# AIM-Harvard/pyradiomics

Measured on AMD Instinct MI355X. Metric: Mvoxels/s for GLCM+GLRLM build, 512^3 vol @32 bins, higher is better.
Workload: dtype u8 levels / u32 counts / f64 out; 1 GPU; GLCM+GLRLM matrix build, 512^3 int32+uint8 volume resident in HBM, 32 grey levels, full mask, 13 angles, uniform levels; one volume per GPU (batch sharding, no collective); size=512, levels=32, dist=uniform, deferred_mode=pipeline

## Files before the change

pyradiomics_amd/csrc/kernels_sweep.h:

```cpp
#pragma once
#include "prad_runtime.h"

namespace prad {

typedef unsigned int u32;
typedef unsigned long long u64;

__global__ void __launch_bounds__(256) pack_levels_kernel(const int *__restrict__ image,
                                                          const uint8_t *__restrict__ mask, long long n, int NX,
                                                          int pitch, int padw, int Ng,
                                                          uint8_t *__restrict__ levels, int *__restrict__ flags,
                                                          int vec_ok, int shift, uint8_t *__restrict__ rowzero = nullptr) {
  const long long tid = (long long)blockIdx.x * blockDim.x + threadIdx.x;
  const long long nthreads = (long long)gridDim.x * blockDim.x;
  const bool linear = (padw == 0 && pitch == NX);
  int bad = 0;
  long long done = 0;
  if (vec_ok) {
    const long long n16 = n >> 4;
    const int upr = NX >> 4;
    const int4 *im4 = reinterpret_cast<const int4 *>(image);
    const uint4 *mk4 = reinterpret_cast<const uint4 *>(mask);
    for (long long t = tid; t < n16; t += nthreads) {
      const uint4 m = mk4[t];
// ... 305 lines not shown
}
template <int LPL, int U, typename W>
__device__ __forceinline__ void steps_plain_group(W (&w)[LPL], const unsigned (&v)[U]) {
#pragma unroll
  for (int k = 0; k < U; k++) step_lines_plain<LPL>(w, v[k]);
}
template <int LPL, int U, bool LONG>
__device__ __forceinline__ void steps_plain_group(Walker<true, true, LONG, true> (&w)[LPL], const unsigned (&v)[U]) {
  unsigned pw = pack_prev<LPL>(w);
#pragma unroll
  for (int k = 0; k < U; k++) {
    step_lines_plain<LPL, LONG>(w, v[k], pw);
    pw = v[k];
  }
  unpack_prev<LPL>(w, pw);
}

template <int LPL, int U, bool CHECK, typename W>
__device__ __forceinline__ bool steps_break_group(W (&w)[LPL], const unsigned (&v)[U], const int (&sb)[U],
                                                  const bool (&uw)[U], int lane4) {
  bool m = false;
#pragma unroll
  for (int k = 0; k < U; k++) {
#pragma unroll
    for (int j = 0; j < LPL; j++) {
      const bool brk = uw[k] || (sb[k] == lane4 + j);
      m |= w[j].template step_brk<CHECK>((int)((v[k] >> (8 * j)) & 0xffu), brk);
    }
  }
  return m;
}
template <bool DO_GLCM, bool DO_GLRLM, bool FUSED>
__device__ __forceinline__ void flush_block_hist(const u32 *lds, const HistLayout &h, int Nr, int slot,
                                                 u32 *__restrict__ glcm_acc, u32 *__restrict__ glrlm_acc) {
  __syncthreads();
  const int Ng = h.Ng;
  if (FUSED) {
    const int Q = Ng + 1, P = (h.RS + 1) * Q;
    u32 *gd = glcm_acc + (size_t)slot * Ng * Ng;
    for (int i = threadIdx.x; i < Ng * Ng; i += blockDim.x) {
      const int p = i / Ng, c = i - p * Ng;
      if (p == c) continue;
      u32 v = 0;
      for (int l = 0; l <= h.RS; l++) v += lds[(p + 1) * P + l * Q + c + 1];
      if (v) atomicAdd(gd + i, v);
    }
    u32 *rd = glrlm_acc + (size_t)slot * Ng * Nr;
    for (int i = threadIdx.x; i < Ng * h.RS; i += blockDim.x) {
      const int p = i / h.RS, l = i - p * h.RS;
      u32 v = 0;
      for (int c = 0; c <= Ng; c++) v += lds[(p + 1) * P + l * Q + c];
      if (v) atomicAdd(rd + (size_t)p * Nr + l, v);
    }
    for (int i = threadIdx.x; i < Ng * h.RL; i += blockDim.x) {
      const int p = i / h.RL, l = h.RS + (i - p * h.RL);
      const u32 v = lds[h.g0 + i];
      if (v && l < Nr) atomicAdd(rd + (size_t)p * Nr + l, v);
    }
    return;
  }
  if (DO_GLCM) {
    u32 *dst = glcm_acc + (size_t)slot * Ng * Ng;
    for (int i = threadIdx.x; i < Ng * Ng; i += blockDim.x) {
      const u32 v = lds[i];
      if (v) atomicAdd(dst + i, v);
    }
  }
  if (DO_GLRLM) {
    const u32 *hr = lds + h.glrlm0;
    u32 *dst = glrlm_acc + (size_t)slot * Ng * Nr;
    for (int i = threadIdx.x; i < h.RS * Ng; i += blockDim.x) {
      const u32 v = hr[i];
      if (v) atomicAdd(dst + (size_t)(i % Ng) * Nr + (i / Ng), v);
    }
  }
}

#ifndef PRAD_SWEEP_UNROLL
#define PRAD_SWEEP_UNROLL 8
#endif

struct __attribute__((packed)) u32_unaligned { u32 v; };
struct __attribute__((packed)) u16_unaligned { unsigned short v; };
template <int LPL>
__device__ __forceinline__ u32 load_lines(const uint8_t *p) {
#ifdef PRAD_DBG_NOLOAD
  const u32 x = (u32)(size_t)p * 2654435761u;
  return ((x >> 7) & 0x1f1f1f1fu) + 0x01010101u;
#else
  if (LPL == 4) return reinterpret_cast<const u32_unaligned *>(p)->v;
// ... 372 lines not shown
```

pyradiomics_amd/csrc/kernels_sweepfw.h:

```cpp
#pragma once
#include "kernels_sweep.h"

namespace prad {

enum FwPhase { FP_INIT, FP_GRAB, FP_CTRL, FP_ISSUE, FP_WAIT_ROWS, FP_WAIT_PACK, FP_GROUP, FP_PACK, FP_SLOW, FP_FLUSH, FP_DRAIN,
               FP_TOTAL, FP_REALTIME, FP_NGROUP, FP_NGROUP_PACK, FP_NSLOW, FP_COUNT };
#ifdef PRAD_FW_STAMPS
__device__ unsigned long long prad_fw_stamps[2 * 8192 * FP_COUNT];
struct FwClock {
  unsigned long long last, first, rt0;
  unsigned acc[FP_COUNT];
  __device__ __forceinline__ void start() {
#pragma unroll
    for (int i = 0; i < FP_COUNT; i++) acc[i] = 0;
    rt0 = __builtin_amdgcn_s_memrealtime();
    first = last = __builtin_readcyclecounter();
  }
  template <int PH>
  __device__ __forceinline__ void lap() {
    const unsigned long long now = __builtin_readcyclecounter();
    acc[PH] += (unsigned)(now - last);
    last = now;
  }
  template <int PH>
// ... 26 lines not shown
  long long sM, sU;
  int CL, pieces;
  int chunks;
  int dom_kind;
};
struct FwSet {
  int count;
  int NX;
  int pitch;
  int nrows;
  int xcd;
  int first_block[PRAD_MAX_SWEEP + 1];
  FwDesc d[PRAD_MAX_SWEEP];
};

struct PackJob {
  const int *image;
  const uint8_t *mask;
  uint8_t *levels;
  uint8_t *levels16;
  uint8_t *rowzero;
  int *flags;
  long long n16;
  int NX, Ng;
  int every;
};

#define PRAD_FW_U 8
#ifndef PRAD_FW_MAXG
#define PRAD_FW_MAXG 4
#endif
#define PRAD_FW_WORK_STRIDE 64
#define PRAD_FW_DOMAINS 8
__host__ __device__ inline size_t fw_lds_bytes(const HistLayout &h) { return 4 * ((size_t)h.words + (size_t)(h.Ng + 1)); }


struct FwTab {
  u32 *rl_long;
  int Nr, P4, Q, lenlim, gB, RL4, RS, RL, dummy0b, alive0, deadmax;
  unsigned Qinv;
  __device__ __forceinline__ void init(const HistLayout &h, int Nr_, u32 *rl_long_) {
    rl_long = rl_long_;
    Nr = Nr_;
    Q = 4 * (h.Ng + 1);
    P4 = (h.RS + 1) * (h.Ng + 1);
    lenlim = (h.RS + 1) * Q;
    RS = h.RS;
    RL = h.RL;
    RL4 = 4 * h.RL;
    gB = Q + 4 * h.g0 - RL4 - 4 * h.RS;
    Qinv = (unsigned)((0x100000000ull + (unsigned)Q - 1) / (unsigned)Q);
    dummy0b = Q + 4 * h.dummy0;
    alive0 = (h.RS + 2) * Q;
    deadmax = (h.RS + 1) * Q;
  }
};

__device__ __noinline__ void fw_long_event(const FwTab &T, int lv, int lb) {
  const int idx = (int)__umulhi((unsigned)lb, T.Qinv);
  if (idx < T.RS + T.RL) {
    lds_bump(T.gB + __mul24(lv, T.RL4) + (idx << 2));
    return;
  }
  const unsigned key = ((unsigned)lv << 20) | (unsigned)idx;
  bool pending = true;
  while (pending) {
// ... 757 lines not shown
      const uint4 *row = reinterpret_cast<const uint4 *>(tile + lane * PRAD_ROW_PITCH);
#pragma unroll
      for (int q = 0; q < 4; q++) {
        const uint4 d = row[q];
        const u32 wds[4] = {d.x, d.y, d.z, d.w};
        const unsigned m = (pw >> 24) ? (unsigned)(s - __mul24((int)(pw >> 24), T.P4)) : 0u;
        if (LONG && __ballot(m + 16 * T.Q > (unsigned)T.lenlim) != 0) {
#pragma unroll 1
          for (int k = 0; k < 4; k++) {
            const u32 c = wds[k], x = __builtin_amdgcn_alignbyte(c, pw, 3);
            const unsigned m4 = (pw >> 24) ? (unsigned)(s - __mul24((int)(pw >> 24), T.P4)) : 0u;
            if (__ballot(m4 + 4 * T.Q > (unsigned)T.lenlim) != 0) {
#pragma unroll
              for (int b = 0; b < 4; b++) fw_checked<LONG>(T, dummy, s, (int)((x >> (8 * b)) & 0xffu), (int)((c >> (8 * b)) & 0xffu), false);
            } else {
              fw_row_word<ZA>(T, one, s, c, x);
            }
            pw = c;
          }
        } else {
#pragma unroll
          for (int k = 0; k < 4; k++) {
            fw_row_word<ZA>(T, one, s, wds[k], __builtin_amdgcn_alignbyte(wds[k], pw, 3));
            pw = wds[k];
          }
        }
      }
      __builtin_amdgcn_wave_barrier();
    }
    fw_checked<LONG>(T, dummy, s, (int)(pw >> 24), 0, false);
  }
}

template <bool LONG>
__global__ void __launch_bounds__(1024) sweep_fw_rows_kernel(const uint8_t *__restrict__ L, long long nrows, int NX, int pitch,
                                                            int slot, int Ng, int Nr, int RS, u32 *__restrict__ glcm_acc,
                                                            u32 *__restrict__ glrlm_acc, int *__restrict__ flags) {
  extern __shared__ u32 lds[];
  if (flags[0]) return;
  const HistLayout h = hist_layout(true, true, true, Ng, RS);
  if ((unsigned)(size_t)((lds_u32 *)lds) != 0u) {
    if (threadIdx.x == 0) atomicExch(flags + 2, 1);
    return;
  }
  for (int i = threadIdx.x; i < h.words + Ng + 1; i += blockDim.x) lds[i] = 0;
  __syncthreads();
  FwTab T;
  T.init(h, Nr, glrlm_acc + (size_t)slot * Ng * Nr);
  if (flags[3] != 0) fw_rows_role<LONG, true>(h, T, lds, L, nrows, NX, pitch, (int)blockIdx.x, (int)gridDim.x);
  else fw_rows_role<LONG, false>(h, T, lds, L, nrows, NX, pitch, (int)blockIdx.x, (int)gridDim.x);
  flush_block_hist<true, true, true>(lds + Ng + 1, h, Nr, slot, glcm_acc, glrlm_acc);
}

template <bool LONG, int K, bool HASPAD, bool PACK>
__global__ void __launch_bounds__(1024) sweep_fw_kernel(FwSet set, PackJob pj, const uint8_t *__restrict__ L,
                                                        const uint8_t *__restrict__ rowzero, int Ng, int Nr, int RS,
                                                        u32 *__restrict__ glcm_acc, u32 *__restrict__ glrlm_acc,
                                                        int *__restrict__ work, int *__restrict__ flags) {
  extern __shared__ u32 lds[];
  int role = 0;
  while (role + 1 < set.count && (int)blockIdx.x >= set.first_block[role + 1]) role++;
  const int bx = (int)blockIdx.x - set.first_block[role], nblocks = set.first_block[role + 1] - set.first_block[role];
  const int wpb = (int)(blockDim.x >> 6);
  const long long pw = __builtin_amdgcn_readfirstlane((int)(blockIdx.x * wpb + (threadIdx.x >> 6)));
  PackWave pk(pj, pw, (long long)gridDim.x * wpb);
  FwClock clk;
  clk.start();
#ifdef PRAD_FW_SETPRIO
  __builtin_amdgcn_s_setprio(PRAD_FW_SETPRIO);
#endif
  if (flags[0] == 0) {
    const bool anyzero = flags[3] != 0;
    const HistLayout h = hist_layout(true, true, true, Ng, RS);
    if ((unsigned)(size_t)((lds_u32 *)lds) != 0u) {
      if (threadIdx.x == 0) atomicExch(flags + 2, 1);
    } else {
      for (int i = threadIdx.x; i < h.words + Ng + 1; i += blockDim.x) lds[i] = 0;
      __syncthreads();
      clk.lap<FP_INIT>();
      const FwDesc &D = set.d[role];
      FwTab T;
      T.init(h, Nr, glrlm_acc + (size_t)D.slot * Ng * Nr);
      int *wk = work + PRAD_FW_WORK_STRIDE * PRAD_FW_DOMAINS * role;
      if (D.dx == 0) {
        FwWave<LONG, K, 0, HASPAD, PACK> w(T, set.NX);
        w.run(D, set.NX, set.pitch, set.nrows, L, rowzero, anyzero, wk, bx, nblocks, pk, pj, set.xcd != 0, clk);
      } else if (D.dx > 0) {
        FwWave<LONG, K, 1, HASPAD, PACK> w(T, set.NX);
        w.run(D, set.NX, set.pitch, set.nrows, L, rowzero, anyzero, wk, bx, nblocks, pk, pj, set.xcd != 0, clk);
      } else {
        FwWave<LONG, K, -1, HASPAD, PACK> w(T, set.NX);
        w.run(D, set.NX, set.pitch, set.nrows, L, rowzero, anyzero, wk, bx, nblocks, pk, pj, set.xcd != 0, clk);
      }
      clk.lap<FP_CTRL>();
      flush_block_hist<true, true, true>(lds + Ng + 1, h, Nr, D.slot, glcm_acc, glrlm_acc);
      clk.lap<FP_FLUSH>();
    }
  }
  if (PACK) pk.drain(pj);
  clk.lap<FP_DRAIN>();
  clk.store(PACK ? 1 : 0);
}

}
```

pyradiomics_amd/csrc/prad_api.hip:

```cpp
#include "prad_runtime.h"
#include "kernels_generic.h"
#include "kernels_pairs.h"
#include "kernels_sweep.h"
#include "kernels_sweepfw.h"
#include "kernels_sweepfw2.h"
#include "kernels_neigh.h"
#include "kernels_glszm.h"
#include "kernels_voxel.h"
#include "kernels_voxslide.h"
#include "kernels_mcc.h"
#include "kernels_voxtex.h"
#include "kernels_binning.h"

#include <algorithm>
#include <atomic>
#include <chrono>
#include <cmath>
#include <condition_variable>
#include <cstdlib>
#include <deque>
#include <limits>
#include <mutex>
#include <thread>

// ... 571 lines not shown
int launch_fw2_khsp(Call &k, const SweepPlan &p, const PackJob &pj, const uint8_t *levels16, int Ng, int Nr, u32 *glcm_acc, u32 *glrlm_acc,
                    int *work, int *flags_d) {
  PRAD_HIP(hipFuncSetAttribute(reinterpret_cast<const void *>(&sweep_fw2_kernel<LNG, K, HASPAD, SKIP1, PACK>),
                               hipFuncAttributeMaxDynamicSharedMemorySize, (int)p.lds_fw2));
  hipLaunchKernelGGL((sweep_fw2_kernel<LNG, K, HASPAD, SKIP1, PACK>), dim3(p.fw_blocks), dim3(1024), p.lds_fw2, k.s, p.fwset, pj, levels16,
                     Ng, Nr, p.RS2, p.fw2_copies, glcm_acc, glrlm_acc, work, flags_d);
  return check_launch("sweep_fw2_kernel");
}
template <bool LNG, int K, bool HASPAD, bool SKIP1>
int launch_fw2_khs(Call &k, const SweepPlan &p, const PackJob &pj, const uint8_t *levels16, int Ng, int Nr, u32 *glcm_acc, u32 *glrlm_acc,
                   int *work, int *flags_d) {
  if (pj.n16 > 0) return launch_fw2_khsp<LNG, K, HASPAD, SKIP1, true>(k, p, pj, levels16, Ng, Nr, glcm_acc, glrlm_acc, work, flags_d);
  return launch_fw2_khsp<LNG, K, HASPAD, SKIP1, false>(k, p, pj, levels16, Ng, Nr, glcm_acc, glrlm_acc, work, flags_d);
}
template <bool LNG, int K>
int launch_fw2_k(Call &k, const SweepPlan &p, const PackJob &pj, const uint8_t *levels16, int Ng, int Nr, u32 *glcm_acc, u32 *glrlm_acc,
                 int *multi, int *flags_d) {
  int *work = multi + 2 * PRAD_MAX_SWEEP + PRAD_FW_WORK_STRIDE;
  if (p.Nx != 64 * K)
    return p.skip1 ? launch_fw2_khs<LNG, K, true, true>(k, p, pj, levels16, Ng, Nr, glcm_acc, glrlm_acc, work, flags_d)
                   : launch_fw2_khs<LNG, K, true, false>(k, p, pj, levels16, Ng, Nr, glcm_acc, glrlm_acc, work, flags_d);
  return p.skip1 ? launch_fw2_khs<LNG, K, false, true>(k, p, pj, levels16, Ng, Nr, glcm_acc, glrlm_acc, work, flags_d)
                 : launch_fw2_khs<LNG, K, false, false>(k, p, pj, levels16, Ng, Nr, glcm_acc, glrlm_acc, work, flags_d);
}
int launch_fw2(Call &k, const SweepPlan &p, const PackJob &pj, const uint8_t *levels16, int Ng, int Nr, u32 *glcm_acc, u32 *glrlm_acc,
               int *multi, int *flags_d) {
  if (p.LONGfw2) return p.fwK == 4 ? launch_fw2_k<true, 4>(k, p, pj, levels16, Ng, Nr, glcm_acc, glrlm_acc, multi, flags_d)
                                 : launch_fw2_k<true, 8>(k, p, pj, levels16, Ng, Nr, glcm_acc, glrlm_acc, multi, flags_d);
  return p.fwK == 4 ? launch_fw2_k<false, 4>(k, p, pj, levels16, Ng, Nr, glcm_acc, glrlm_acc, multi, flags_d)
                    : launch_fw2_k<false, 8>(k, p, pj, levels16, Ng, Nr, glcm_acc, glrlm_acc, multi, flags_d);
}

template <bool LNG>
int launch_fw_rows(Call &k, const SweepPlan &p, const uint8_t *levels, int Ng, int Nr, u32 *glcm_acc, u32 *glrlm_acc, int *flags_d) {
  const long long nrows = (long long)p.Nz * p.Ny, groups = nrows >= 4096 ? ((nrows + 511) / 512) * 8 : (nrows + 63) / 64;
  const int wpb = p.fw_rows_threads / 64;
  const unsigned gx = (unsigned)std::max<long long>(1, std::min<long long>((groups + wpb - 1) / wpb, (long long)cu_count()));
  PRAD_HIP(hipFuncSetAttribute(reinterpret_cast<const void *>(&sweep_fw_rows_kernel<LNG>),
                               hipFuncAttributeMaxDynamicSharedMemorySize, (int)p.lds_fw_rows));
  hipLaunchKernelGGL((sweep_fw_rows_kernel<LNG>), dim3(gx), dim3(p.fw_rows_threads), p.lds_fw_rows, k.s, levels, nrows, p.Nx,
                     p.pitch, p.row_slot, Ng, Nr, p.RSfw_rows, glcm_acc, glrlm_acc, flags_d);
  return check_launch("sweep_fw_rows_kernel");
}

template <bool LNG>
int launch_fw2_rows(Call &k, const SweepPlan &p, const uint8_t *levels16, int Ng, int Nr, u32 *glcm_acc, u32 *glrlm_acc, int *flags_d) {
  const long long nrows = (long long)p.Nz * p.Ny, groups = nrows >= 4096 ? ((nrows + 511) / 512) * 8 : (nrows + 63) / 64;
  const int wpb = p.fw2r_waves;
  const unsigned gx = (unsigned)std::max<long long>(1, std::min<long long>((groups + wpb - 1) / wpb, (long long)cu_count()));
  PRAD_HIP(hipFuncSetAttribute(reinterpret_cast<const void *>(&sweep_fw2_rows_kernel<LNG>),
                               hipFuncAttributeMaxDynamicSharedMemorySize, (int)p.lds_fw2_rows));
  hipLaunchKernelGGL((sweep_fw2_rows_kernel<LNG>), dim3(gx), dim3(64 * wpb), p.lds_fw2_rows, k.s, levels16, nrows, p.Nx, p.pitch16,
                     p.row_slot, Ng, Nr, p.RS2r, p.fw2r_copies, glcm_acc, glrlm_acc, flags_d);
  return check_launch("sweep_fw2_rows_kernel");
}

template <bool G, bool R, bool LNG, bool F>
int launch_rows(Call &k, const SweepPlan &p, const uint8_t *levels, int Ng, int Nr, u32 *glcm_acc, u32 *glrlm_acc,
                int *multi) {
  const long long nrows = (long long)p.Nz * p.Ny;
  const long long groups = (nrows + 63) / 64;
  const int wpb = kRowsThreads / 64;
  const int per_cu = std::max(1, std::min(2048 / kRowsThreads, (int)(160 * 1024 / p.lds_bytes_rows)));
  const unsigned gx = (unsigned)std::max<long long>(1, std::min<long long>((groups + wpb - 1) / wpb, (long long)cu_count() * per_cu));
  PRAD_HIP(hipFuncSetAttribute(reinterpret_cast<const void *>(&sweep_rows_kernel<G, R, LNG, F>),
                               hipFuncAttributeMaxDynamicSharedMemorySize, (int)p.lds_bytes_rows));
  hipLaunchKernelGGL((sweep_rows_kernel<G, R, LNG, F>), dim3(gx), dim3(kRowsThreads), p.lds_bytes_rows, k.s, levels,
                     nrows, p.Nx, p.pitch, p.row_slot, Ng, Nr, p.RSr, glcm_acc, glrlm_acc, multi, k.flags_d);
  return check_launch("sweep_rows_kernel");
}

__global__ void __launch_bounds__(256) zero3_kernel(u32 *__restrict__ a, size_t na, u32 *__restrict__ b, size_t nb,
                                                    u32 *__restrict__ c3, size_t nc) {
  const size_t t = (size_t)blockIdx.x * blockDim.x + threadIdx.x, nt = (size_t)gridDim.x * blockDim.x;
  uint4 *a4 = reinterpret_cast<uint4 *>(a);
  for (size_t i = t; i < na / 4; i += nt) a4[i] = make_uint4(0, 0, 0, 0);
  for (size_t i = (na & ~(size_t)3) + t; i < na; i += nt) a[i] = 0;
  for (size_t i = t; i < nb; i += nt) b[i] = 0;
  for (size_t i = t; i < nc; i += nt) c3[i] = 0;
}

struct VolState {
  bool valid = false;
  SweepPlan p;
  int Ng = 0, Nr = 0, Na = 0;
  double *glcm = nullptr, *glrlm = nullptr;
  uint8_t *levels = nullptr, *rowzero = nullptr;
  uint8_t *levels16 = nullptr;
  u32 *acc = nullptr, *glcm_acc = nullptr, *glrlm_acc = nullptr;
  int *multi = nullptr;
  int *flags_d = nullptr;
  bool packed_inline = false;
  int lane = -1;
};

bool fin_side() {
  static const bool on = getenv("PRAD_FINALIZE_STREAM") != nullptr && atoi(getenv("PRAD_FINALIZE_STREAM")) != 0;
  return on;
}
int fin_wait_for_lane(hipStream_t s, int lane);

int vol_prepare(Call &k, const SweepPlan &p, int Ng, int Nr, double *glcm, double *glrlm, VolState &v) {
  Context &c = *k.c;
  if (fin_side() && c.lane >= 0) PRAD_TRY(fin_wait_for_lane(k.s, c.lane));
  v.lane = c.lane;
  v.valid = true;
  v.p = p;
  v.Ng = Ng;
  v.Nr = Nr;
  v.Na = k.Na;
  v.glcm = glcm;
  v.glrlm = glrlm;
  v.flags_d = k.flags_d;
  const long long nrows = (long long)p.Nz * p.Ny;
  v.levels = nullptr;
  if (!(p.fw2 && p.fw2_rows && p.lines.count > 0 && p.row_slot >= 0) || getenv("PRAD_FW2_KEEP8")) {
    PRAD_TRY(c.get<uint8_t>("levels", (size_t)nrows * p.pitch + 1024, &v.levels));
    v.levels += 512;
  }
  v.levels16 = nullptr;
  if (p.fw2) {
    PRAD_TRY(c.get<uint8_t>("levels16", (size_t)nrows * p.pitch16 + 4096, &v.levels16));
    v.levels16 += 2048;
  }
  const size_t nglcm = glcm ? (size_t)k.Na * Ng * Ng : 0, nglrlm = glrlm ? (size_t)k.Na * Ng * Nr : 0;
  const size_t nctl = 2 * PRAD_MAX_SWEEP + (size_t)PRAD_FW_WORK_STRIDE * (PRAD_FW_DOMAINS * PRAD_MAX_SWEEP + 1);
  PRAD_TRY(c.get<u32>("sweep_acc", nglcm + nglrlm + nctl, &v.acc));
  v.glcm_acc = v.acc;
  v.glrlm_acc = v.acc + nglcm;
  v.multi = (int *)(v.acc + nglcm + nglrlm);
  v.rowzero = nullptr;
  if (p.fw) PRAD_TRY(c.get<uint8_t>("rowzero", (size_t)nrows + 64, &v.rowzero));
  const size_t acc_w = nglcm + nglrlm + nctl, rz_w = v.rowzero ? ((size_t)nrows + 3) / 4 : 0;
  const size_t total_w = acc_w + rz_w + 4;
  const unsigned gx = (unsigned)std::max<size_t>(1, std::min<size_t>((total_w / 4 + 255) / 256, 1024));
  hipLaunchKernelGGL(zero3_kernel, dim3(gx), dim3(256), 0, k.s, v.acc, acc_w, reinterpret_cast<u32 *>(v.rowzero), rz_w,
                     reinterpret_cast<u32 *>(v.flags_d), (size_t)4);
  return check_launch("zero3_kernel");
}

bool pipeline_volume(const SweepPlan &p, bool glcm, bool glrlm) {
  if (!(p.ok && p.lines.count > 0 && glcm && glrlm)) return false;
  return (p.fw && p.fused) || (p.fw2 && !getenv("PRAD_FW2_LANES"));
}
bool pack_inline_ok(const Call &k, const VolState &v) {
  if (!(v.glcm && v.glrlm && v.p.pitch == v.p.Nx && v.p.padw == 0 && (k.g.n % 16) == 0 &&
        ((((uintptr_t)k.image) | ((uintptr_t)k.mask) | ((uintptr_t)v.levels)) & 15) == 0))
    return false;
  if (k.g.n >= (1LL << 31)) return false;
  if (v.p.fw2) return v.levels16 && v.p.pitch16 == 2 * v.p.Nx && (((uintptr_t)v.levels16) & 15) == 0;
  return v.p.fw && v.p.fused;
}

PackJob make_pack_job(const Call &k, const VolState &v, const VolState *host) {
  PackJob j;
  memset(&j, 0, sizeof(j));
  j.image = k.image;
  j.mask = k.mask;
  j.levels = v.levels;
  j.levels16 = v.p.fw2 ? v.levels16 : nullptr;
  j.rowzero = v.rowzero;
  j.flags = v.flags_d;
  j.n16 = k.g.n / 16;
  j.NX = v.p.Nx;
  j.Ng = v.Ng;
  double groups = 0, waves = 16.0;
  if (host) {
    for (int i = 0; i < host->p.fwset.count; i++) groups += (double)host->p.fwset.d[i].NM * host->p.fwset.d[i].NU / PRAD_FW_U;
    waves = 16.0 * std::max(1, host->p.fw_blocks);
  }
// ... 16 lines not shown
    return check_launch("pack_levels16_kernel");
  }
  const int vec_ok = p.vec_rows && ((((uintptr_t)k.image) | ((uintptr_t)k.mask) | ((uintptr_t)v.levels)) & 15) == 0;
  const unsigned gx = (unsigned)std::max<long long>(1, std::min<long long>((k.g.n / 16 + 255) / 256, 4096));
  const int shift = (v.glcm && v.glrlm && p.fused) ? PRAD_FUSED_SHIFT : 0;
  hipLaunchKernelGGL(pack_levels_kernel, dim3(gx), dim3(256), 0, k.s, k.image, k.mask, k.g.n, p.Nx, p.pitch, p.padw,
                     v.Ng, v.levels, v.flags_d, vec_ok, shift, v.rowzero);
  return check_launch("pack_levels_kernel");
}

template <bool G, bool R, bool F>
int launch_sweeps(Call &k, const VolState &v, const PackJob &pj) {
  const SweepPlan &p = v.p;
  if (p.lines.count > 0 && p.fw && G && R && F) {
    static const bool rows_side = getenv("PRAD_ROWS_STREAM") != nullptr;
    if (rows_side && p.row_slot >= 0) {
      static thread_local hipStream_t side = nullptr;
      static thread_local hipEvent_t e0 = nullptr, e1 = nullptr;
      if (!side) {
        int lo = 0, hi = 0;
        PRAD_HIP(hipDeviceGetStreamPriorityRange(&lo, &hi));
        PRAD_HIP(hipStreamCreateWithPriority(&side, hipStreamNonBlocking, getenv("PRAD_ROWS_STREAM_PRIO") ? atoi(getenv("PRAD_ROWS_STREAM_PRIO")) : lo));
        PRAD_HIP(hipEventCreateWithFlags(&e0, hipEventDisableTiming));
        PRAD_HIP(hipEventCreateWithFlags(&e1, hipEventDisableTiming));
      }
      PRAD_HIP(hipEventRecord(e0, k.s));
      PRAD_HIP(hipStreamWaitEvent(side, e0, 0));
      {
        Timed t(*k.c, "sweep", k.s);
        PRAD_TRY(launch_fw(k, p, pj, v.levels, v.rowzero, v.Ng, v.Nr, v.glcm_acc, v.glrlm_acc, v.multi, v.flags_d));
      }
      Call k2 = k;
      k2.s = side;
      if (p.RSfw_rows < v.Nr) PRAD_TRY(launch_fw_rows<true>(k2, p, v.levels, v.Ng, v.Nr, v.glcm_acc, v.glrlm_acc, v.flags_d));
      else PRAD_TRY(launch_fw_rows<false>(k2, p, v.levels, v.Ng, v.Nr, v.glcm_acc, v.glrlm_acc, v.flags_d));
      PRAD_HIP(hipEventRecord(e1, side));
      PRAD_HIP(hipStreamWaitEvent(k.s, e1, 0));
      return PRAD_OK;
    }
    {
      Timed t(*k.c, "sweep", k.s);
      PRAD_TRY(launch_fw(k, p, pj, v.levels, v.rowzero, v.Ng, v.Nr, v.glcm_acc, v.glrlm_acc, v.multi, v.flags_d));
    }
    if (p.row_slot >= 0) {
      Timed t(*k.c, "rows", k.s);
      if (p.RSfw_rows < v.Nr) PRAD_TRY(launch_fw_rows<true>(k, p, v.levels, v.Ng, v.Nr, v.glcm_acc, v.glrlm_acc, v.flags_d));
      else PRAD_TRY(launch_fw_rows<false>(k, p, v.levels, v.Ng, v.Nr, v.glcm_acc, v.glrlm_acc, v.flags_d));
    }
    return PRAD_OK;
  }
  if (p.fw2 && G && R && !F && p.lines.count > 0) {
    {
      Timed t(*k.c, "sweep", k.s);
      PRAD_TRY(launch_fw2(k, p, pj, v.levels16, v.Ng, v.Nr, v.glcm_acc, v.glrlm_acc, v.multi, v.flags_d));
    }
    if (p.row_slot >= 0) {
      Timed t(*k.c, "rows", k.s);
      if (p.fw2_rows) {
        if (p.LONGfw2r) PRAD_TRY(launch_fw2_rows<true>(k, p, v.levels16, v.Ng, v.Nr, v.glcm_acc, v.glrlm_acc, v.flags_d));
        else PRAD_TRY(launch_fw2_rows<false>(k, p, v.levels16, v.Ng, v.Nr, v.glcm_acc, v.glrlm_acc, v.flags_d));
      } else if (p.LONGr) {
        PRAD_TRY((launch_rows<G, R, true, F>(k, p, v.levels, v.Ng, v.Nr, v.glcm_acc, v.glrlm_acc, v.multi)));
      } else {
        PRAD_TRY((launch_rows<G, R, false, F>(k, p, v.levels, v.Ng, v.Nr, v.glcm_acc, v.glrlm_acc, v.multi)));
      }
    }
    return PRAD_OK;
  }
  Timed t(*k.c, "sweep", k.s);
  if (p.lines.count > 0) {
    if (R && p.LONG) PRAD_TRY((launch_lines<G, R, true, F>(k, p, v.levels, v.Ng, v.Nr, v.glcm_acc, v.glrlm_acc, v.multi)));
    else PRAD_TRY((launch_lines<G, R, false, F>(k, p, v.levels, v.Ng, v.Nr, v.glcm_acc, v.glrlm_acc, v.multi)));
  }
  if (p.row_slot >= 0) {
    if (R && p.LONGr) PRAD_TRY((launch_rows<G, R, true, F>(k, p, v.levels, v.Ng, v.Nr, v.glcm_acc, v.glrlm_acc, v.multi)));
    else PRAD_TRY((launch_rows<G, R, false, F>(k, p, v.levels, v.Ng, v.Nr, v.glcm_acc, v.glrlm_acc, v.multi)));
  }
  return PRAD_OK;
}

int vol_sweep(Call &k, const VolState &v, const PackJob &pj) {
  if (pj.n16 > 0 && !pipeline_volume(v.p, v.glcm != nullptr, v.glrlm != nullptr))
    return fail(PRAD_E_ARG, "internal: a pack job needs a fixed-window host launch");
  if (pj.n16 > 0 && (pj.levels16 != nullptr) != v.p.fw2)
    return fail(PRAD_E_ARG, "internal: the pack job's layout is not the host launch's");
  if (v.glcm && v.glrlm && v.p.fused) return launch_sweeps<true, true, true>(k, v, pj);
  if (v.glcm && v.glrlm) return launch_sweeps<true, true, false>(k, v, pj);
  if (v.glcm) return launch_sweeps<true, false, false>(k, v, pj);
  return launch_sweeps<false, true, false>(k, v, pj);
}

__global__ void latch_flags_kernel(const int *__restrict__ flags, int *__restrict__ sticky) {
  if (flags[0] || flags[2]) sticky[0] = 1;
}

__global__ void latch_any_flag_kernel(const int *__restrict__ flags, int *__restrict__ sticky) {
  if (flags[0] || flags[1] || flags[2]) sticky[0] = 1;
}
int latch_neigh(Context &c, Call &k) {
  int *sticky = nullptr;
  PRAD_TRY(c.get<int>("deferred_sticky", 16, &sticky));
  hipLaunchKernelGGL(latch_any_flag_kernel, dim3(1), dim3(1), 0, k.s, (const int *)k.flags_d, sticky);
  return check_launch("latch_any_flag_kernel");
}

int vol_finalize(Call &k, const VolState &v, int *sticky) {
  Context &c = *k.c;
  const SweepPlan &p = v.p;
  const int Ng = v.Ng, Nr = v.Nr, Na = v.Na;
  double *glcm = v.glcm, *glrlm = v.glrlm;
  bool latched = false;
  {
    Timed t(c, "finalize", k.s);
    const bool runs_diag = p.fused || p.fw2;
    if (p.fw2 && p.skip1 && p.lines.count > 0 && !(glcm && glrlm && p.row_slot >= 0))
      return fail(PRAD_E_UNSUPPORTED, "sweep plan derives runs of length 1 but the call cannot restore them");
    if (glcm && glrlm && runs_diag) {
      const int nb1 = (int)blocks_for((long long)Ng * Ng * Na), nb2 = (Ng * Na + 3) / 4;
      hipLaunchKernelGGL(finalize_glcm_diag_kernel, dim3(nb1 + nb2), dim3(256), 0, k.s, v.glcm_acc, v.glrlm_acc, Ng, Nr, Na, nb1,
                         glcm, v.multi, (p.fw2 && p.skip1 && p.lines.count > 0) ? p.row_slot : -1);
      PRAD_TRY(check_launch("finalize_glcm_diag_kernel"));
    } else if (glcm) {
      hipLaunchKernelGGL(finalize_glcm_kernel, dim3(blocks_for((long long)Ng * Ng * Na)), dim3(256), 0, k.s,
                         v.glcm_acc, v.glrlm_acc, Ng, Nr, Na, p.fused ? 1 : 0, glcm);
      PRAD_TRY(check_launch("finalize_glcm_kernel"));
    }
    if (glrlm && runs_diag) {
      if (!glcm) {
        hipLaunchKernelGGL(glcm_diag_resolve_kernel, dim3(Ng, Na), dim3(64), 0, k.s, v.glcm_acc, v.glrlm_acc, Ng, Nr, Na,
                           glcm, v.multi);
        PRAD_TRY(check_launch("glcm_diag_resolve_kernel"));
      }
      if (v.levels)
        hipLaunchKernelGGL(multi_check_kernel<uint8_t>, dim3(128, Na), dim3(256), 0, k.s, p.aset, (const uint8_t *)v.levels, p.Nz, p.Ny,
                           p.Nx, p.pitch, v.multi);
      else
        hipLaunchKernelGGL(multi_check_kernel<unsigned short>, dim3(128, Na), dim3(256), 0, k.s, p.aset,
                           reinterpret_cast<const unsigned short *>(v.levels16), p.Nz, p.Ny, p.Nx, p.pitch16 / 2, v.multi);
      PRAD_TRY(check_launch("multi_check_kernel"));
    }
    if (glrlm) {
      hipLaunchKernelGGL(finalize_glrlm_kernel, dim3(blocks_for((long long)Ng * Nr * Na)), dim3(256), 0, k.s,
                         v.glrlm_acc, v.multi, Ng, Nr, Na, glrlm, (const int *)v.flags_d, sticky);
      PRAD_TRY(check_launch("finalize_glrlm_kernel"));
      latched = sticky != nullptr;
    }
  }
  if (sticky && !latched) {
    hipLaunchKernelGGL(latch_flags_kernel, dim3(1), dim3(1), 0, k.s, v.flags_d, sticky);
    PRAD_TRY(check_launch("latch_flags_kernel"));
  }
  return PRAD_OK;
}

int sweep_glcm_glrlm(Call &k, const SweepPlan &p, int Ng, int Nr, double *glcm, double *glrlm, bool *used) {
  Context &c = *k.c;
  VolState v;
  PRAD_TRY(vol_prepare(k, p, Ng, Nr, glcm, glrlm, v));
  PRAD_TRY(vol_pack_standalone(k, v));
  PackJob pj;
  memset(&pj, 0, sizeof(pj));
  PRAD_TRY(vol_sweep(k, v, pj));
  int *sticky = nullptr;
  if (c.deferred) PRAD_TRY(c.get<int>("deferred_sticky", 16, &sticky));
  PRAD_TRY(vol_finalize(k, v, sticky));
  if (c.deferred) {
    *used = true;
    return PRAD_OK;
  }
  PRAD_TRY(read_flags(k));
  *used = (k.flags_h[0] == 0 && k.flags_h[2] == 0);
  return PRAD_OK;
}

struct PipeState {
  VolState pending;
  hipStream_t s = nullptr;
  unsigned long long seq = 0;
  hipEvent_t ev = nullptr;
  int mode = -1;
  hipStream_t fin = nullptr;
  hipEvent_t fin_in = nullptr, fin_all = nullptr, fin_done[4] = {};
  bool fin_used[4] = {};
};
PipeState &pipe_state() {
  static thread_local PipeState p;
  return p;
}
bool pipeline_mode() {
  PipeState &ps = pipe_state();
  if (ps.mode < 0) {
    const char *e = getenv("PRAD_DEFERRED_MODE");
    ps.mode = (e && strcmp(e, "lanes") == 0) ? 0 : 1;
  }
  return ps.mode == 1;
}
int pipeline_sticky(Context &c, int **sticky) { return c.get<int>("deferred_sticky", 16, sticky); }

int pipeline_retire(Context &c, hipStream_t s, const PackJob &pj) {
  PipeState &ps = pipe_state();
  if (ps.s != s) {
    if (!ps.ev) PRAD_HIP(hipEventCreateWithFlags(&ps.ev, hipEventDisableTiming));
    PRAD_HIP(hipEventRecord(ps.ev, ps.s));
    PRAD_HIP(hipStreamWaitEvent(s, ps.ev, 0));
// ... 1554 lines not shown
```

pyradiomics_amd/csrc/prad_runtime.h:

```cpp
#pragma once

#include <hip/hip_runtime.h>
#include <stdint.h>
#include <stdio.h>
#include <stdarg.h>
#include <string.h>
#include <stdlib.h>
#include <string>
#include <vector>
#include <map>

#include "../../include/pyradiomics_amd.h"

namespace prad {

struct ErrorState {
  char msg[512];
  ErrorState() { msg[0] = 0; }
};
inline ErrorState &err_state() {
  static thread_local ErrorState e;
  return e;
}
inline int fail(int code, const char *fmt, ...) {
  va_list ap;
  va_start(ap, fmt);
  vsnprintf(err_state().msg, sizeof(err_state().msg), fmt, ap);
  va_end(ap);
  return code;
}

#define PRAD_HIP(call)                                                                              \
  do {                                                                                              \
    hipError_t e_ = (call);                                                                         \
    if (e_ != hipSuccess)                                                                           \
      return ::prad::fail(e_ == hipErrorOutOfMemory ? PRAD_E_NOMEM : PRAD_E_HIP, "%s failed: %s (%s:%d)", \
                          #call, hipGetErrorString(e_), __FILE__, __LINE__);                        \
  } while (0)

struct DevBuf {
  void *p = nullptr;
  size_t cap = 0;
};

struct KernelTime {
  std::string family;
  hipEvent_t a, b;
};

#define PRAD_MAX_LANES 4
#define PRAD_ARENA_BYTES (4u << 20)

struct Context {
  int device = 0;
  bool device_set = false;
  hipStream_t own_stream = nullptr;
  std::map<std::string, DevBuf> bufs;
  std::map<std::string, DevBuf> pinned;
  std::vector<KernelTime> times;
  std::vector<hipEvent_t> event_pool;
  size_t events_used = 0;
  hipEvent_t call_a = nullptr, call_b = nullptr;
  bool call_timed = false;
  const char *last_path = "none";
  const char *last_variant = "none";
  bool deferred = false;
  bool timing_accumulate = false;
  std::string timing_only;
  std::vector<KernelTime> all_times;
  std::vector<std::pair<hipEvent_t, hipEvent_t>> all_calls;
  std::map<std::string, std::vector<int>> angles_cached;
  int workspace = 0;
  int lanes = 0;
  int lane = -1;
  unsigned long long lane_seq = 0;
  hipStream_t lane_stream[PRAD_MAX_LANES] = {};
  hipEvent_t lane_in[PRAD_MAX_LANES] = {};
  long long glszm_nzones = 0;
  int glszm_nvox = 0;
  int glszm_max_region = 0;
  std::vector<long long> glszm_zone_offsets;

  int ensure_device() {
    if (!device_set) {
      int n = 0;
      hipError_t e = hipGetDeviceCount(&n);
      if (e != hipSuccess || n <= 0)
        return fail(PRAD_E_HIP, "no HIP device visible (hipGetDeviceCount: %s) -- this library has no CPU fallback",
                    hipGetErrorString(e));
      device_set = true;
    }
    PRAD_HIP(hipSetDevice(device));
    if (!own_stream) PRAD_HIP(hipStreamCreateWithFlags(&own_stream, hipStreamNonBlocking));
    return PRAD_OK;
  }

  std::string key(const char *name) const {
    std::string k(name);
    if (k.compare(0, 9, "deferred_") != 0) {
      if (lane >= 0) k += "#" + std::to_string(lane);
      if (workspace) k += "~" + std::to_string(workspace);
    }
    return k + "@" + std::to_string(device);
  }
  bool has(const char *name) const { return bufs.find(key(name)) != bufs.end(); }
  std::vector<int> &angle_cache() { return angles_cached[key("angles")]; }
  int lane_begin(hipStream_t user, hipStream_t *s) {
    if (lanes == 0) {
      const char *e = getenv("PRAD_LANES");
      lanes = e ? atoi(e) : 2;
      lanes = lanes < 1 ? 1 : (lanes > PRAD_MAX_LANES ? PRAD_MAX_LANES : lanes);
    }
    if (lanes == 1) return PRAD_OK;
    const int l = (int)(lane_seq++ % (unsigned)lanes);
    if (!lane_stream[l]) {
      PRAD_HIP(hipStreamCreateWithFlags(&lane_stream[l], hipStreamNonBlocking));
      PRAD_HIP(hipEventCreateWithFlags(&lane_in[l], hipEventDisableTiming));
    }
    PRAD_HIP(hipEventRecord(lane_in[l], user));
    PRAD_HIP(hipStreamWaitEvent(lane_stream[l], lane_in[l], 0));
    lane = l;
    *s = lane_stream[l];
    return PRAD_OK;
  }
  int lanes_join(hipStream_t s) {
    for (int l = 0; l < PRAD_MAX_LANES; l++)
      if (lane_stream[l]) {
        PRAD_HIP(hipEventRecord(lane_in[l], lane_stream[l]));
        PRAD_HIP(hipStreamWaitEvent(s, lane_in[l], 0));
      }
    return PRAD_OK;
  }
  int lanes_sync() {
    for (int l = 0; l < PRAD_MAX_LANES; l++)
      if (lane_stream[l]) PRAD_HIP(hipStreamSynchronize(lane_stream[l]));
    return PRAD_OK;
  }

  int get(const char *name, size_t bytes, void **out) {
    DevBuf &b = bufs[key(name)];
    if (b.cap < bytes) {
      if (b.p) (void)hipFree(b.p);
      b.p = nullptr;
      b.cap = 0;
      size_t want = bytes + bytes / 8 + 256;
      hipError_t e = hipMalloc(&b.p, want);
      if (e != hipSuccess) {
        b.p = nullptr;
        return fail(PRAD_E_NOMEM, "hipMalloc(%zu) for workspace '%s' failed: %s", want, name, hipGetErrorString(e));
      }
      b.cap = want;
    }
    *out = b.p;
    return PRAD_OK;
  }
  template <typename T>
  int get(const char *name, size_t count, T **out) {
    void *p = nullptr;
    int rc = get(name, count * sizeof(T), &p);
    *out = (T *)p;
    return rc;
  }
  int get_pinned(const char *name, size_t bytes, void **out) {
    DevBuf &b = pinned[workspace ? std::string(name) + "~" + std::to_string(workspace) : std::string(name)];
    if (b.cap < bytes) {
      if (b.p) (void)hipHostFree(b.p);
      b.p = nullptr;
      b.cap = 0;
      hipError_t e = hipHostMalloc(&b.p, bytes + 256, hipHostMallocDefault);
      if (e != hipSuccess) {
        b.p = nullptr;
        return fail(PRAD_E_NOMEM, "hipHostMalloc(%zu) failed: %s", bytes, hipGetErrorString(e));
      }
      b.cap = bytes + 256;
    }
    *out = b.p;
    return PRAD_OK;
  }

  char *arena = nullptr;
  size_t arena_pos = 0;
  int arena_alloc(size_t bytes, void **out) {
    bytes = (bytes + 63) & ~(size_t)63;
    if (bytes > PRAD_ARENA_BYTES / 4) return fail(PRAD_E_ARG, "result arena: %zu bytes in one allocation", bytes);
// ... 177 lines not shown
```

Measured before the change: 286,600 Mvoxels/s.

## Fuse finalize into rows kernel and skip redundant accumulator zeroing

Moves the per-angle finalize (u32-to-f64 conversion, GLRLM run-length-1 handling, diagonal fill) into the tail of the rows sweep kernel and a small finish_x_kernel that also clears the accumulators, rowzero and control words in place. Because the finish pass leaves the workspace zeroed, the zero3 launch at the start of the next call is skipped when host-side generation tracking says the buffers are still clean. A multi-voxel-per-line detection (multi flags, line scans) replaces the earlier diagonal/column-0 logic. This removes separate launches and a memset pass, but adds scanning work and cross-call state that could go stale.

```diff
diff --git a/pyradiomics_amd/csrc/kernels_sweep.h b/pyradiomics_amd/csrc/kernels_sweep.h
--- a/pyradiomics_amd/csrc/kernels_sweep.h
+++ b/pyradiomics_amd/csrc/kernels_sweep.h
@@ -361,30 +361,46 @@
 }
 template <bool DO_GLCM, bool DO_GLRLM, bool FUSED>
 __device__ __forceinline__ void flush_block_hist(const u32 *lds, const HistLayout &h, int Nr, int slot,
-                                                 u32 *__restrict__ glcm_acc, u32 *__restrict__ glrlm_acc) {
+                                                 u32 *__restrict__ glcm_acc, u32 *__restrict__ glrlm_acc,
+                                                 int *__restrict__ multi = nullptr) {
   __syncthreads();
   const int Ng = h.Ng;
   if (FUSED) {
     const int Q = Ng + 1, P = (h.RS + 1) * Q;
+    bool found = false;
     u32 *gd = glcm_acc + (size_t)slot * Ng * Ng;
     for (int i = threadIdx.x; i < Ng * Ng; i += blockDim.x) {
       const int p = i / Ng, c = i - p * Ng;
       if (p == c) continue;
       u32 v = 0;
       for (int l = 0; l <= h.RS; l++) v += lds[(p + 1) * P + l * Q + c + 1];
-      if (v) atomicAdd(gd + i, v);
+      if (v) {
+        atomicAdd(gd + i, v);
+        found = true;
+      }
     }
     u32 *rd = glrlm_acc + (size_t)slot * Ng * Nr;
     for (int i = threadIdx.x; i < Ng * h.RS; i += blockDim.x) {
       const int p = i / h.RS, l = i - p * h.RS;
       u32 v = 0;
       for (int c = 0; c <= Ng; c++) v += lds[(p + 1) * P + l * Q + c];
-      if (v) atomicAdd(rd + (size_t)p * Nr + l, v);
+      if (v) {
+        atomicAdd(rd + (size_t)p * Nr + l, v);
+        found = found || l > 0;
+      }
     }
     for (int i = threadIdx.x; i < Ng * h.RL; i += blockDim.x) {
       const int p = i / h.RL, l = h.RS + (i - p * h.RL);
       const u32 v = lds[h.g0 + i];
       if (v && l < Nr) atomicAdd(rd + (size_t)p * Nr + l, v);
+      found = found || v != 0;
+    }
+    if (multi) {
+      for (int i = threadIdx.x; i < Ng * Q; i += blockDim.x) {
+        const int p = i / Q, c = i - p * Q;
+        found = found || lds[(p + 1) * P + h.RS * Q + c] != 0;
+      }
+      if (found) multi[slot] = 1;
     }
     return;
   }
diff --git a/pyradiomics_amd/csrc/kernels_sweepfw.h b/pyradiomics_amd/csrc/kernels_sweepfw.h
--- a/pyradiomics_amd/csrc/kernels_sweepfw.h
+++ b/pyradiomics_amd/csrc/kernels_sweepfw.h
@@ -82,6 +82,10 @@
 #endif
 #define PRAD_FW_WORK_STRIDE 64
 #define PRAD_FW_DOMAINS 8
+#define PRAD_FW_CTL_FLAGS (2 * PRAD_MAX_SWEEP)
+#define PRAD_FW_CTL_VERDICT (2 * PRAD_MAX_SWEEP + 4)
+#define PRAD_FW_CTL_WORK (2 * PRAD_MAX_SWEEP + PRAD_FW_WORK_STRIDE)
+#define PRAD_FW_CTL_WORDS (2 * PRAD_MAX_SWEEP + PRAD_FW_WORK_STRIDE * (PRAD_FW_DOMAINS * PRAD_MAX_SWEEP + 1))
 __host__ __device__ inline size_t fw_lds_bytes(const HistLayout &h) { return 4 * ((size_t)h.words + (size_t)(h.Ng + 1)); }
 
 
@@ -905,12 +909,123 @@
   }
 }
 
+struct FinishJob {
+  int on;
+  int Na, Nz, Ny;
+  int *multi;
+  double *glcm_out, *glrlm_out;
+  AngleSet A;
+};
+
+__device__ __forceinline__ bool finish_in_scope(int a, int only, int skip) { return only >= 0 ? a == only : a != skip; }
+
+__device__ __forceinline__ void finish_slots(const FinishJob &J, u32 *glcm_acc, u32 *glrlm_acc, int Ng, int Nr, int only, int skip,
+                                             bool own_col0, int bx, int nb) {
+  const int Na = J.Na;
+  const long long total = (long long)Ng * Ng * Na, nthreads = (long long)nb * blockDim.x;
+  for (long long idx = (long long)(nb - 1 - bx) * blockDim.x + threadIdx.x; idx < total; idx += nthreads) {
+    const int a = (int)(idx % Na);
+    const long long ij = idx / Na;
+    const int i = (int)(ij / Ng), j = (int)(ij - (long long)i * Ng);
+    if (i == j || !finish_in_scope(a, only, skip)) continue;
+    u32 *src = glcm_acc + (size_t)a * Ng * Ng + ij;
+    J.glcm_out[idx] = (double)*src;
+    *src = 0;
+  }
+  const int lane = threadIdx.x & 63, wave = threadIdx.x >> 6, wpb = blockDim.x >> 6;
+  for (long long q = bx + (long long)wave * nb; q < (long long)Ng * Na; q += (long long)nb * wpb) {
+    const int a = (int)(q / Ng), i = (int)(q - (long long)a * Ng);
+    if (!finish_in_scope(a, only, skip)) continue;
+    const bool keep0 = own_col0 || J.multi[a] != 1;
+    u32 *row = glrlm_acc + ((size_t)a * Ng + i) * Nr;
+    unsigned long long pairs = 0;
+    for (int r = lane; r < Nr; r += 64) {
+      if (r == 0 && keep0) continue;
+      const u32 v = row[r];
+      pairs += (unsigned long long)r * v;
+      J.glrlm_out[((size_t)i * Nr + r) * Na + a] = (double)v;
+      row[r] = 0;
+    }
+    for (int o = 32; o > 0; o >>= 1) pairs += __shfl_xor(pairs, o);
+    if (lane == 0) J.glcm_out[((size_t)i * Ng + i) * Na + a] = (double)pairs;
+  }
+}
+
+__device__ __forceinline__ void finish_scan_lines(const FinishJob &J, int a, const uint8_t *__restrict__ L, int NX, int pitch, int bx,
+                                                  int nb) {
+  const int Nz = J.Nz, Ny = J.Ny;
+  const int dz = J.A.off[a][0], dy = J.A.off[a][1], dx = J.A.off[a][2];
+  const long long n = (long long)Nz * Ny * NX, plane = (long long)Ny * NX, stride = (long long)nb * blockDim.x;
+  volatile int *m = J.multi + a;
+  int it = 0;
+  for (long long i = (long long)bx * blockDim.x + threadIdx.x; i < n; i += stride, it++) {
+    if ((it & 31) == 0 && *m != 0) return;
+    int z = (int)(i / plane);
+    const int r = (int)(i - (long long)z * plane);
+    int y = r / NX, x = r - y * NX;
+    const int pz = z - dz, py = y - dy, px = x - dx;
+    if ((unsigned)pz < (unsigned)Nz && (unsigned)py < (unsigned)Ny && (unsigned)px < (unsigned)NX) continue;
+    int cnt = 0;
+    while ((unsigned)z < (unsigned)Nz && (unsigned)y < (unsigned)Ny && (unsigned)x < (unsigned)NX) {
+      cnt += L[((long long)z * Ny + y) * pitch + x] != 0;
+      if (cnt > 1) {
+        *m = 2;
+        return;
+      }
+      z += dz; y += dy; x += dx;
+    }
+  }
+}
+
+__device__ __forceinline__ bool finish_scan_rows(const uint8_t *__restrict__ L, long long nrows, int NX, int pitch, volatile u32 *flag) {
+  const int lane = threadIdx.x & 63, wave = threadIdx.x >> 6, wpb = blockDim.x >> 6;
+  __syncthreads();
+  if (threadIdx.x == 0) *flag = 0;
+  __syncthreads();
+  for (long long r0 = (long long)wave * 4; r0 < nrows; r0 += (long long)wpb * 4) {
+    if (*flag) break;
+    int cnt[4] = {0, 0, 0, 0};
+    for (int x = lane * 4; x < NX; x += 256) {
+      const int keep = NX - x;
+      const u32 km = keep >= 4 ? 0xffffffffu : ((1u << (8 * keep)) - 1u);
+#pragma unroll
+      for (int k = 0; k < 4; k++) {
+        if (r0 + k >= nrows) continue;
+        const u32 w = *reinterpret_cast<const u32 *>(L + (r0 + k) * pitch + x) & km;
+        cnt[k] += __popc((((w & 0x7f7f7f7fu) + 0x7f7f7f7fu) | w) & 0x80808080u);
+      }
+    }
+    bool hit = false;
+#pragma unroll
+    for (int k = 0; k < 4; k++) hit = hit || __ballot(cnt[k] > 1) != 0 || __popcll(__ballot(cnt[k] == 1)) > 1;
+    if (hit) {
+      *flag = 1;
+      break;
+    }
+  }
+  __syncthreads();
+  return *flag != 0;
+}
+
 template <bool LONG>
 __global__ void __launch_bounds__(1024) sweep_fw_rows_kernel(const uint8_t *__restrict__ L, long long nrows, int NX, int pitch,
                                                             int slot, int Ng, int Nr, int RS, u32 *__restrict__ glcm_acc,
-                                                            u32 *__restrict__ glrlm_acc, int *__restrict__ flags) {
+                                                            u32 *__restrict__ glrlm_acc, int *__restrict__ flags, FinishJob fin) {
   extern __shared__ u32 lds[];
-  if (flags[0]) return;
+  const int irregular = flags[0];
+  if (fin.on) {
+    unsigned open = 0;
+#pragma unroll
+    for (int a = 0; a < PRAD_MAX_SWEEP; a++) open |= (fin.multi[a] == 0 ? 1u : 0u) << a;
+    open &= (1u << fin.Na) - 1u;
+    open &= ~(1u << slot);
+    finish_slots(fin, glcm_acc, glrlm_acc, Ng, Nr, -1, slot, false, (int)blockIdx.x, (int)gridDim.x);
+    if (open != 0 && !irregular) {
+      for (int a = 0; a < fin.Na; a++)
+        if ((open >> a) & 1u) finish_scan_lines(fin, a, L, NX, pitch, (int)blockIdx.x, (int)gridDim.x);
+    }
+  }
+  if (irregular) return;
   const HistLayout h = hist_layout(true, true, true, Ng, RS);
   if ((unsigned)(size_t)((lds_u32 *)lds) != 0u) {
     if (threadIdx.x == 0) atomicExch(flags + 2, 1);
@@ -922,7 +1037,49 @@
   T.init(h, Nr, glrlm_acc + (size_t)slot * Ng * Nr);
   if (flags[3] != 0) fw_rows_role<LONG, true>(h, T, lds, L, nrows, NX, pitch, (int)blockIdx.x, (int)gridDim.x);
   else fw_rows_role<LONG, false>(h, T, lds, L, nrows, NX, pitch, (int)blockIdx.x, (int)gridDim.x);
-  flush_block_hist<true, true, true>(lds + Ng + 1, h, Nr, slot, glcm_acc, glrlm_acc);
+  flush_block_hist<true, true, true>(lds + Ng + 1, h, Nr, slot, glcm_acc, glrlm_acc, fin.on ? fin.multi : nullptr);
+}
+
+__global__ void __launch_bounds__(512) finish_x_kernel(FinishJob fin, const uint8_t *__restrict__ L, int NX, int pitch, int slot, int Ng,
+                                                       int Nr, u32 *__restrict__ glcm_acc, u32 *__restrict__ glrlm_acc,
+                                                       u32 *__restrict__ rowzero_w, long long rz_words, int *__restrict__ ctl,
+                                                       int nctl, int *__restrict__ flags, int *__restrict__ verdict,
+                                                       int *__restrict__ sticky) {
+  __shared__ u32 flag;
+  __shared__ int kept[PRAD_MAX_SWEEP];
+  if (blockIdx.x == 0) {
+    const int f0 = flags[0], f2 = flags[2];
+    int f = 0;
+    if (threadIdx.x < 4) f = flags[threadIdx.x];
+    if ((int)threadIdx.x < fin.Na) {
+      const int m = fin.multi[threadIdx.x];
+      kept[threadIdx.x] = ((int)threadIdx.x == slot) ? (m != 0 || f0 != 0) : (m == 1 ? -1 : (m != 0));
+    }
+    __syncthreads();
+    if (!kept[slot]) {
+      const bool hit = finish_scan_rows(L, (long long)fin.Nz * fin.Ny, NX, pitch, &flag);
+      if (threadIdx.x == 0) kept[slot] = hit ? 1 : 0;
+      __syncthreads();
+    }
+    for (int q = threadIdx.x; q < Ng * fin.Na; q += blockDim.x) {
+      const int a = q / Ng, i = q - a * Ng;
+      if (kept[a] < 0) continue;
+      u32 *src = glrlm_acc + ((size_t)a * Ng + i) * Nr;
+      fin.glrlm_out[((size_t)i * Nr) * fin.Na + a] = kept[a] ? (double)*src : 0.0;
+      *src = 0;
+    }
+    if (threadIdx.x == 0 && sticky && (f0 != 0 || f2 != 0)) sticky[0] = 1;
+    if (threadIdx.x < 4) {
+      verdict[threadIdx.x] = f;
+      flags[threadIdx.x] = 0;
+    }
+    for (int i = threadIdx.x; i < nctl; i += blockDim.x)
+      if (ctl + i < verdict || ctl + i >= verdict + 4) ctl[i] = 0;
+    return;
+  }
+  const int bx = (int)blockIdx.x - 1, nb = (int)gridDim.x - 1;
+  finish_slots(fin, glcm_acc, glrlm_acc, Ng, Nr, slot, -1, true, bx, nb);
+  for (long long i = (long long)bx * blockDim.x + threadIdx.x; i < rz_words; i += (long long)nb * blockDim.x) rowzero_w[i] = 0;
 }
 
 template <bool LONG, int K, bool HASPAD, bool PACK>
@@ -937,6 +1094,8 @@
   const int wpb = (int)(blockDim.x >> 6);
   const long long pw = __builtin_amdgcn_readfirstlane((int)(blockIdx.x * wpb + (threadIdx.x >> 6)));
   PackWave pk(pj, pw, (long long)gridDim.x * wpb);
+  int *multi = work - PRAD_FW_CTL_WORK;
+  asm volatile("" : "+v"(multi));
   FwClock clk;
   clk.start();
 #ifdef PRAD_FW_SETPRIO
@@ -966,7 +1125,7 @@
         w.run(D, set.NX, set.pitch, set.nrows, L, rowzero, anyzero, wk, bx, nblocks, pk, pj, set.xcd != 0, clk);
       }
       clk.lap<FP_CTRL>();
-      flush_block_hist<true, true, true>(lds + Ng + 1, h, Nr, D.slot, glcm_acc, glrlm_acc);
+      flush_block_hist<true, true, true>(lds + Ng + 1, h, Nr, D.slot, glcm_acc, glrlm_acc, multi);
       clk.lap<FP_FLUSH>();
     }
   }
diff --git a/pyradiomics_amd/csrc/prad_api.hip b/pyradiomics_amd/csrc/prad_api.hip
--- a/pyradiomics_amd/csrc/prad_api.hip
+++ b/pyradiomics_amd/csrc/prad_api.hip
@@ -627,14 +627,15 @@
 }
 
 template <bool LNG>
-int launch_fw_rows(Call &k, const SweepPlan &p, const uint8_t *levels, int Ng, int Nr, u32 *glcm_acc, u32 *glrlm_acc, int *flags_d) {
+int launch_fw_rows(Call &k, const SweepPlan &p, const uint8_t *levels, int Ng, int Nr, u32 *glcm_acc, u32 *glrlm_acc, int *flags_d,
+                   const FinishJob &fin) {
   const long long nrows = (long long)p.Nz * p.Ny, groups = nrows >= 4096 ? ((nrows + 511) / 512) * 8 : (nrows + 63) / 64;
   const int wpb = p.fw_rows_threads / 64;
   const unsigned gx = (unsigned)std::max<long long>(1, std::min<long long>((groups + wpb - 1) / wpb, (long long)cu_count()));
   PRAD_HIP(hipFuncSetAttribute(reinterpret_cast<const void *>(&sweep_fw_rows_kernel<LNG>),
                                hipFuncAttributeMaxDynamicSharedMemorySize, (int)p.lds_fw_rows));
   hipLaunchKernelGGL((sweep_fw_rows_kernel<LNG>), dim3(gx), dim3(p.fw_rows_threads), p.lds_fw_rows, k.s, levels, nrows, p.Nx,
-                     p.pitch, p.row_slot, Ng, Nr, p.RSfw_rows, glcm_acc, glrlm_acc, flags_d);
+                     p.pitch, p.row_slot, Ng, Nr, p.RSfw_rows, glcm_acc, glrlm_acc, flags_d, fin);
   return check_launch("sweep_fw_rows_kernel");
 }
 
@@ -687,7 +688,39 @@
   int *flags_d = nullptr;
   bool packed_inline = false;
   int lane = -1;
+  bool finish = false;
+  int *verdict = nullptr;
+  std::string setkey;
 };
+
+bool finish_route(const SweepPlan &p, bool glcm, bool glrlm) {
+  static const bool chain = getenv("PRAD_FINISH_CHAIN") != nullptr && atoi(getenv("PRAD_FINISH_CHAIN")) != 0;
+  static const bool side = getenv("PRAD_ROWS_STREAM") != nullptr;
+  return !chain && !side && p.ok && p.fw && p.fused && p.lines.count > 0 && p.row_slot >= 0 && glcm && glrlm;
+}
+struct SetState {
+  bool clean = false;
+  unsigned long long acc_gen = 0, rz_gen = 0;
+  size_t nglcm = 0, nglrlm = 0, rz_w = 0;
+};
+std::map<std::string, SetState> &set_states() {
+  static thread_local std::map<std::string, SetState> m;
+  return m;
+}
+FinishJob make_finish_job(const VolState &v) {
+  FinishJob j;
+  memset(&j, 0, sizeof(j));
+  if (!v.finish) return j;
+  j.on = 1;
+  j.Na = v.Na;
+  j.Nz = v.p.Nz;
+  j.Ny = v.p.Ny;
+  j.multi = v.multi;
+  j.glcm_out = v.glcm;
+  j.glrlm_out = v.glrlm;
+  j.A = v.p.aset;
+  return j;
+}
 
 bool fin_side() {
   static const bool on = getenv("PRAD_FINALIZE_STREAM") != nullptr && atoi(getenv("PRAD_FINALIZE_STREAM")) != 0;
@@ -719,7 +752,7 @@
     v.levels16 += 2048;
   }
   const size_t nglcm = glcm ? (size_t)k.Na * Ng * Ng : 0, nglrlm = glrlm ? (size_t)k.Na * Ng * Nr : 0;
-  const size_t nctl = 2 * PRAD_MAX_SWEEP + (size_t)PRAD_FW_WORK_STRIDE * (PRAD_FW_DOMAINS * PRAD_MAX_SWEEP + 1);
+  const size_t nctl = PRAD_FW_CTL_WORDS;
   PRAD_TRY(c.get<u32>("sweep_acc", nglcm + nglrlm + nctl, &v.acc));
   v.glcm_acc = v.acc;
   v.glrlm_acc = v.acc + nglcm;
@@ -727,10 +760,28 @@
   v.rowzero = nullptr;
   if (p.fw) PRAD_TRY(c.get<uint8_t>("rowzero", (size_t)nrows + 64, &v.rowzero));
   const size_t acc_w = nglcm + nglrlm + nctl, rz_w = v.rowzero ? ((size_t)nrows + 3) / 4 : 0;
+  v.finish = finish_route(p, glcm != nullptr, glrlm != nullptr) && !fin_side();
+  v.verdict = nullptr;
+  if (v.finish) {
+    v.flags_d = v.multi + PRAD_FW_CTL_FLAGS;
+    v.verdict = v.multi + PRAD_FW_CTL_VERDICT;
+  }
+  v.setkey = c.key("sweep_acc");
+  SetState &st = set_states()[v.setkey];
+  const unsigned long long acc_gen = c.gen("sweep_acc"), rz_gen = v.rowzero ? c.gen("rowzero") : 0;
+  const bool still_clean = st.clean && st.acc_gen == acc_gen && st.rz_gen == rz_gen && st.nglcm == nglcm && st.nglrlm == nglrlm &&
+                           st.rz_w == rz_w;
+  st.clean = false;
+  st.acc_gen = acc_gen;
+  st.rz_gen = rz_gen;
+  st.nglcm = nglcm;
+  st.nglrlm = nglrlm;
+  st.rz_w = rz_w;
+  if (v.finish && still_clean) return PRAD_OK;
   const size_t total_w = acc_w + rz_w + 4;
   const unsigned gx = (unsigned)std::max<size_t>(1, std::min<size_t>((total_w / 4 + 255) / 256, 1024));
   hipLaunchKernelGGL(zero3_kernel, dim3(gx), dim3(256), 0, k.s, v.acc, acc_w, reinterpret_cast<u32 *>(v.rowzero), rz_w,
-                     reinterpret_cast<u32 *>(v.flags_d), (size_t)4);
+                     reinterpret_cast<u32 *>(k.flags_d), (size_t)4);
   return check_launch("zero3_kernel");
 }
 
@@ -813,8 +864,9 @@
       }
       Call k2 = k;
       k2.s = side;
-      if (p.RSfw_rows < v.Nr) PRAD_TRY(launch_fw_rows<true>(k2, p, v.levels, v.Ng, v.Nr, v.glcm_acc, v.glrlm_acc, v.flags_d));
-      else PRAD_TRY(launch_fw_rows<false>(k2, p, v.levels, v.Ng, v.Nr, v.glcm_acc, v.glrlm_acc, v.flags_d));
+      const FinishJob nofin = make_finish_job(VolState());
+      if (p.RSfw_rows < v.Nr) PRAD_TRY(launch_fw_rows<true>(k2, p, v.levels, v.Ng, v.Nr, v.glcm_acc, v.glrlm_acc, v.flags_d, nofin));
+      else PRAD_TRY(launch_fw_rows<false>(k2, p, v.levels, v.Ng, v.Nr, v.glcm_acc, v.glrlm_acc, v.flags_d, nofin));
       PRAD_HIP(hipEventRecord(e1, side));
       PRAD_HIP(hipStreamWaitEvent(k.s, e1, 0));
       return PRAD_OK;
@@ -825,8 +877,9 @@
     }
     if (p.row_slot >= 0) {
       Timed t(*k.c, "rows", k.s);
-      if (p.RSfw_rows < v.Nr) PRAD_TRY(launch_fw_rows<true>(k, p, v.levels, v.Ng, v.Nr, v.glcm_acc, v.glrlm_acc, v.flags_d));
-      else PRAD_TRY(launch_fw_rows<false>(k, p, v.levels, v.Ng, v.Nr, v.glcm_acc, v.glrlm_acc, v.flags_d));
+      const FinishJob fin = make_finish_job(v);
+      if (p.RSfw_rows < v.Nr) PRAD_TRY(launch_fw_rows<true>(k, p, v.levels, v.Ng, v.Nr, v.glcm_acc, v.glrlm_acc, v.flags_d, fin));
+      else PRAD_TRY(launch_fw_rows<false>(k, p, v.levels, v.Ng, v.Nr, v.glcm_acc, v.glrlm_acc, v.flags_d, fin));
     }
     return PRAD_OK;
   }
@@ -891,6 +944,17 @@
   const int Ng = v.Ng, Nr = v.Nr, Na = v.Na;
   double *glcm = v.glcm, *glrlm = v.glrlm;
   bool latched = false;
+  if (v.finish) {
+    Timed t(c, "finalize", k.s);
+    const FinishJob fin = make_finish_job(v);
+    const long long rz_words = ((long long)p.Nz * p.Ny + 3) / 4;
+    hipLaunchKernelGGL(finish_x_kernel, dim3(1 + 32), dim3(512), 0, k.s, fin, (const uint8_t *)v.levels, p.Nx, p.pitch, p.row_slot,
+                       Ng, Nr, v.glcm_acc, v.glrlm_acc, reinterpret_cast<u32 *>(v.rowzero), rz_words, v.multi,
+                       (int)PRAD_FW_CTL_WORDS, v.flags_d, v.verdict, sticky);
+    PRAD_TRY(check_launch("finish_x_kernel"));
+    set_states()[v.setkey].clean = true;
+    return PRAD_OK;
+  }
   {
     Timed t(c, "finalize", k.s);
     const bool runs_diag = p.fused || p.fw2;
@@ -949,8 +1013,14 @@
     *used = true;
     return PRAD_OK;
   }
-  PRAD_TRY(read_flags(k));
+  if (v.finish) {
+    PRAD_HIP(hipMemcpyAsync(k.flags_h, v.verdict, sizeof(int) * 4, hipMemcpyDeviceToHost, k.s));
+    PRAD_HIP(hipStreamSynchronize(k.s));
+  } else {
+    PRAD_TRY(read_flags(k));
+  }
   *used = (k.flags_h[0] == 0 && k.flags_h[2] == 0);
+  if (v.finish && !*used) PRAD_HIP(hipMemsetAsync(k.flags_d, 0, sizeof(int) * 4, k.s));
   return PRAD_OK;
 }
 
diff --git a/pyradiomics_amd/csrc/prad_runtime.h b/pyradiomics_amd/csrc/prad_runtime.h
--- a/pyradiomics_amd/csrc/prad_runtime.h
+++ b/pyradiomics_amd/csrc/prad_runtime.h
@@ -41,6 +41,7 @@
 struct DevBuf {
   void *p = nullptr;
   size_t cap = 0;
+  unsigned long long gen = 0;
 };
 
 struct KernelTime {
@@ -104,6 +105,10 @@
     return k + "@" + std::to_string(device);
   }
   bool has(const char *name) const { return bufs.find(key(name)) != bufs.end(); }
+  unsigned long long gen(const char *name) const {
+    auto it = bufs.find(key(name));
+    return it == bufs.end() ? 0ull : it->second.gen;
+  }
   std::vector<int> &angle_cache() { return angles_cached[key("angles")]; }
   int lane_begin(hipStream_t user, hipStream_t *s) {
     if (lanes == 0) {
@@ -150,6 +155,8 @@
         return fail(PRAD_E_NOMEM, "hipMalloc(%zu) for workspace '%s' failed: %s", want, name, hipGetErrorString(e));
       }
       b.cap = want;
+      static unsigned long long next_gen = 0;
+      b.gen = ++next_gen;
     }
     *out = b.p;
     return PRAD_OK;
```

New measurement: 287,500 Mvoxels/s, median of 6. Within noise of the previous version (+0.3%).
